# antonilo/unsupervised_detection

Measured on AMD Instinct MI355X. Metric: frame-pairs/sec per adversarial step, DAVIS 480p batch4, 1/2/4/8 GPU, higher is better.
Workload: dtype f32

## Files before the change

unsupervised_detection_amd/csrc/api_plan.hip:

```cpp
#include <stdlib.h>
#include <string.h>

#include "conv_host.h"
#include "elementwise.h"
#include "plan.h"

using namespace udet;

struct udet_plan {
  Plan* p;
};

extern "C" {

int udet_plan_create(const udet_config* c, udet_plan** out) {
  if (!c || !out) { set_error("plan_create: null argument"); return UDET_ERR_ARG; }
  Config k;
  k.batch = c->batch; k.in_h = c->in_h; k.in_w = c->in_w; k.img_h = c->img_h; k.img_w = c->img_w;
  k.flow_normalizer = c->flow_normalizer; k.cbn = c->cbn; k.epsilon = c->epsilon;
  k.lr = c->lr; k.beta1 = c->beta1; k.beta2 = c->beta2; k.adam_eps = c->adam_eps; k.clip = c->clip;
  k.noise_seed = c->noise_seed;
  k.conv_fp16 = c->conv_fp16 ? 1 : 0;
  Plan* P = plan_build(k);
  if (!P) return UDET_ERR_SHAPE;
// ... 53 lines not shown
}

int udet_pack_pwc(udet_plan* h, const float* w_pwc, void* ws, void* stream) {
  return plan_pack_pwc(h->p, w_pwc, (float*)ws, (hipStream_t)stream);
}
int udet_pack_trainable(udet_plan* h, const float* w_gen, const float* w_rec, void* ws, void* stream) {
  return plan_pack_trainable(h->p, w_gen, w_rec, (float*)ws, (hipStream_t)stream);
}
int udet_pwc_forward(udet_plan* h, const float* img1, const float* img2, void* ws, void* stream) {
  return plan_pwc_forward(h->p, img1, img2, (float*)ws, (hipStream_t)stream);
}
int udet_forward_from_flow(udet_plan* h, int ncalls, void* ws, void* stream) {
  UDET_TRY(plan_check_overflow(h->p, false));
  if (ncalls < 0 || ncalls > 3) { set_error("forward: ncalls must be 0..3"); return UDET_ERR_ARG; }
  return plan_forward(h->p, nullptr, nullptr, ncalls, (float*)ws, (hipStream_t)stream);
}
int udet_generator_forward(udet_plan* h, void* ws, void* stream) {
  UDET_TRY(plan_generator_forward(h->p, (float*)ws, (hipStream_t)stream));
  return plan_recover_forward(h->p, 0, (float*)ws, (hipStream_t)stream);
}
int udet_generator_layers(udet_plan* h, void* ws, void* stream) {
  h->p->ev_next = 0;
  UDET_TRY(plan_generator_layers(h->p, (float*)ws, (hipStream_t)stream));
  return plan_recover_forward(h->p, 0, (float*)ws, (hipStream_t)stream);
}
int udet_recover_forward(udet_plan* h, int n, void* ws, void* stream) {
  if (n < 1 || n > 3) { set_error("recover_forward: n must be 1..3 (multiples of the plan batch)"); return UDET_ERR_ARG; }
  return plan_recover_forward(h->p, n, (float*)ws, (hipStream_t)stream, true);
}
int udet_forward(udet_plan* h, const float* img1, const float* img2, int ncalls, void* ws, void* stream) {
  UDET_TRY(plan_check_overflow(h->p, false));
  if (ncalls < 0 || ncalls > 3) { set_error("forward: ncalls must be 0..3"); return UDET_ERR_ARG; }
  if (!img1 || !img2) { set_error("forward: null image pointer"); return UDET_ERR_ARG; }
  return plan_forward(h->p, img1, img2, ncalls, (float*)ws, (hipStream_t)stream);
}
int udet_prefetch_flow(udet_plan* h, const float* img1, const float* img2, void* ws, void* stream) {
  if (!img1 || !img2) { set_error("prefetch_flow: null image pointer"); return UDET_ERR_ARG; }
  return plan_prefetch(h->p, img1, img2, (float*)ws, (hipStream_t)stream);
}
int udet_prefetch_consume(udet_plan* h, void* ws, void* stream) {
  return plan_prefetch_consume(h->p, (float*)ws, (hipStream_t)stream);
}
int udet_forward_prefetched(udet_plan* h, int ncalls, void* ws, void* stream) {
  UDET_TRY(plan_check_overflow(h->p, false));
  if (ncalls < 0 || ncalls > 3) { set_error("forward: ncalls must be 0..3"); return UDET_ERR_ARG; }
  return plan_forward(h->p, nullptr, nullptr, ncalls, (float*)ws, (hipStream_t)stream, true);
}
int udet_backward(udet_plan* h, int which, const float* w_gen, const float* w_rec, float* g_gen, float* g_rec, void* ws,
                  void* stream) {
  UDET_TRY(plan_check_overflow(h->p, false));
  if (which < 1 || which > 3) { set_error("backward: which must be 1 (generator), 2 (recover) or 3 (both)"); return UDET_ERR_ARG; }
  return plan_backward(h->p, which, w_gen, w_rec, g_gen, g_rec, (float*)ws, (hipStream_t)stream);
}
int udet_apply(udet_plan* h, int net, float* w, float* g, float* m, float* v, void* ws, void* stream) {
  return plan_apply(h->p, net, w, g, m, v, (float*)ws, (hipStream_t)stream);
}
int udet_train_step(udet_plan* h, int which, const float* img1, const float* img2, float* w_gen, float* w_rec, float* g_gen,
                    float* g_rec, float* m_gen, float* v_gen, float* m_rec, float* v_rec, void* ws, void* stream) {
  UDET_TRY(udet_pack_trainable(h, w_gen, w_rec, ws, stream));
  UDET_TRY(udet_forward(h, img1, img2, 3, ws, stream));
  UDET_TRY(udet_backward(h, which, w_gen, w_rec, g_gen, g_rec, ws, stream));
  if (which & 1) UDET_TRY(udet_apply(h, NET_GEN, w_gen, g_gen, m_gen, v_gen, ws, stream));
  if (which & 2) UDET_TRY(udet_apply(h, NET_REC, w_rec, g_rec, m_rec, v_rec, ws, stream));
  return UDET_OK;
}

int udet_autotune(udet_plan* h, const float* w_gen, const float* w_rec, float* g_gen, float* g_rec, void* ws_, void* stream) {
  Plan* P = h->p;
  float* ws = (float*)ws_;
  hipStream_t s = (hipStream_t)stream;
  if (!P->pwc_packed) { set_error("autotune: pack the PWC-Net and trainable weights first"); return UDET_ERR_ARG; }
  const size_t lo = P->packed_floats, hi = P->small_off;
  UDET_TRY(launch_fill_uniform(ws + lo, (long)(hi - lo), 0x5eedull, -0.5f, 0.5f, s));
  const size_t img_floats = (size_t)P->cfg.batch * P->cfg.in_h * P->cfg.in_w * 3;
  if (P->wgrad_floats < 2 * img_floats) { set_error("autotune: workspace too small for the probe images"); return UDET_ERR_ARG; }
  const float* img1 = ws + P->wgrad_off[0];
  const float* img2 = img1 + img_floats;
  const bool was_concurrent = P->concurrent;
  P->concurrent = false;
  conv_set_tuning(1);
  wgrad_set_tuning(1);
  int rc = udet_forward(h, img1, img2, 3, ws_, stream);
  if (rc == UDET_OK) rc = udet_backward(h, 3, w_gen, w_rec, g_gen, g_rec, ws_, stream);
  conv_set_tuning(0);
  wgrad_set_tuning(0);
  P->concurrent = was_concurrent;
  UDET_HIP(hipMemsetAsync(ws + lo, 0, (hi - lo) * sizeof(float), s));
  UDET_HIP(hipStreamSynchronize(s));
  return rc;
}
int udet_tuned_shapes(void) { return tuned_shapes(); }
int udet_tune_save(const char* path) {
  FILE* f = path ? fopen(path, "w") : nullptr;
  if (!f) { set_error("tune_save: cannot open %s", path ? path : "(null)"); return UDET_ERR_ARG; }
  fprintf(f, "udet-tune 2 abi %d\n", UDET_TUNE_ABI);
  tune_dump(f);
  fclose(f);
  return UDET_OK;
}
int udet_tune_load(const char* path) {
  FILE* f = path ? fopen(path, "r") : nullptr;
  if (!f) { set_error("tune_load: cannot open %s", path ? path : "(null)"); return UDET_ERR_ARG; }
  char line[256];
  int n = 0, ver = 0, abi = -1;
  if (!fgets(line, sizeof(line), f) || sscanf(line, "udet-tune %d abi %d", &ver, &abi) != 2 || ver != 2 || abi != UDET_TUNE_ABI) {
    fclose(f);
    set_error("tune_load: %s is not a udet-tune 2 file of this build (abi %d)", path, UDET_TUNE_ABI);
    return UDET_ERR_ARG;
  }
  while (fgets(line, sizeof(line), f)) n += tune_put_line(line) ? 1 : 0;
  fclose(f);
  return n;
}

int udet_profile_begin(udet_plan* h) {
  for (auto* r : h->p->prof) delete r;
  h->p->prof.clear();
  h->p->profiling = true;
  return UDET_OK;
}
int udet_profile_end(udet_plan* h, double* out, int ncat, void* stream) {
  Plan* P = h->p;
  P->profiling = false;
  g_launch_sink = nullptr;
  UDET_HIP(hipStreamSynchronize((hipStream_t)stream));
  for (int i = 0; i < ncat * 5; ++i) out[i] = 0.0;
  FILE* dump = nullptr;
  if (const char* path = getenv("UDET_PROF_DUMP")) dump = fopen(path, "a");
  for (auto* r : P->prof) {
    float wall = 0.f;
    (void)hipEventElapsedTime(&wall, r->a, r->b);
    double kern = 0.0;
    std::string each;
    for (int k = 0; k < r->sink.n; ++k) {
      float ms = 0.f;
      if (hipEventElapsedTime(&ms, r->kev[2 * k], r->kev[2 * k + 1]) == hipSuccess) kern += ms;
      char buf[32];
      snprintf(buf, sizeof(buf), "%s%.1f", k ? "+" : "", ms * 1e3f);
      each += buf;
      (void)hipEventDestroy(r->kev[2 * k]);
      (void)hipEventDestroy(r->kev[2 * k + 1]);
    }
    if (r->sink.n == 0) kern = wall;
    if (dump)
      fprintf(dump, "%d,%s,%.4f,%.4f,%.4f,%.4f,%d,%s,%.4f\n", r->cat, r->name.c_str(), kern, r->flops * 1e-9, r->bytes * 1e-6, wall, r->sink.n,
              each.c_str(), r->flops * r->mfma_scale * 1e-9);
    if (r->cat < ncat) {
      out[r->cat * 5 + 0] += 1.0;
      out[r->cat * 5 + 1] += kern;
      out[r->cat * 5 + 2] += r->flops;
      out[r->cat * 5 + 3] += r->bytes;
      out[r->cat * 5 + 4] += wall;
    }
    (void)hipEventDestroy(r->a);
    (void)hipEventDestroy(r->b);
    delete r;
  }
  if (dump) fclose(dump);
  P->prof.clear();
  return UDET_OK;
}

int udet_generator_backward(udet_plan* h, const float* w_gen, float* g_gen, void* ws, void* stream) {
  if (!w_gen || !g_gen) { set_error("generator_backward: null argument"); return UDET_ERR_ARG; }
  return plan_backward(h->p, 1, w_gen, nullptr, g_gen, nullptr, (float*)ws, (hipStream_t)stream);
}
// ... 22 lines not shown
```

unsupervised_detection_amd/csrc/elementwise.h:

```cpp
#pragma once
#include "common.h"
namespace udet {
int launch_resize_bilinear_fwd(const float* x, int ldx, int x_coff, int N, int H, int W, float* y, int ldy, int y_coff,
                               int OH, int OW, int C, float mul, float div, hipStream_t s);
int launch_resize_bilinear_bwd(const float* dy, int ldy, int y_coff, int N, int OH, int OW, float* dx, int ldx, int x_coff,
                               int H, int W, int C, int accumulate, hipStream_t s);
int launch_upb_ring(const float* x, int ld, int N, int H, int W, float* xh, hipStream_t s);
int launch_upb_ring_fold(const float* dxh, int ld, int N, int H, int W, float* dx, hipStream_t s);
int launch_share_samples(float* buf, long P, int ld, int coff, int C, int copies, hipStream_t s);
int launch_fold_samples(float* buf, long P, int ld, int coff, int C, int copies, hipStream_t s);
int launch_emit_du(const float* d, const float* a, float* u, long P, int ld, int coff, int C, int act, float alpha, hipStream_t s);
int launch_pool2x2_sum(const float* du, float* dx, int N, int H, int W, int C, hipStream_t s);
int launch_pack_pwc_input(const float* i1, const float* i2, float* x8, long P, hipStream_t s);
int launch_gen_input(const float* img, const float* f, double* part, float* gin, int B, long HW, hipStream_t s);
size_t flow_stats_doubles(int B);
int launch_mask_rec_inputs(const float* logits, const float* f, float* mask, float* fin, long P, int ncalls, hipStream_t s);
int launch_pack_imgin(const float* img, float* imgin, long P, int ncalls, hipStream_t s);
int launch_losses(const float* f, const float* mask, const float* pred, long HW, int B, float cbn, float eps,
                  float num_pixels, float* part, float* losses, float* coef, float* sums, hipStream_t s);
size_t loss_part_floats(int B);
int launch_rec_loss_bwd(const float* f, const float* mask, const float* pred, float* dpred, long BHW, float cbn,
                        float inv_np, hipStream_t s);
int launch_gen_loss_bwd(const float* f, const float* mask, const float* pred, const float* coef, float* dpred,
                        float* dmask, long HW, int B, float cbn, hipStream_t s);
int launch_mask_bwd(const float* dmask, const float* dfin, const float* f, const float* mask, float* dlogits, long P,
                    hipStream_t s);
int launch_grad_absmean(const float* g, const long* seg_off, const long* seg_len, int nvars, float* vmean, float thresh,
                        float* out, hipStream_t s);
int launch_adam(float* w, float* g, float* m, float* v, long n, float lr_t, float b1, float b2, float eps, float clip,
                const float* flag, uint64_t seed, uint64_t step, hipStream_t s, int mode = 0, const int* skip = nullptr);
int launch_nonfinite_count(const float* g, long n, int* out, hipStream_t s);
int launch_flow_normalize(const float* f, double* part, float* out, int B, long HW, hipStream_t s);
int launch_charbonnier(const float* gt, const float* pred, const float* mask, int mc, int B, long HW, float cbn, float* part,
                       float* out, hipStream_t s);
int launch_crop_flip_resize(const void* src, int src_u8, int nearest, int N, int H, int W, int C, const int* prm, float* dst, int OH,
                            int OW, float div, float add, hipStream_t s);
int launch_crop_flip_resize_ragged(const void* src, int src_u8, int nearest, int N, int C, const long long* offsets, const int* hw,
                                   const int* prm, float* dst, int OH, int OW, float div, float add, hipStream_t s);
int launch_mask_stats(const float* pred, const float* gt, int N, int H, int W, float threshold, float gt_threshold, double* out,
                      hipStream_t s);
int launch_boundary_stats(const float* pred, const float* gt, const double* stats8, int N, int H, int W, float threshold,
                          float gt_threshold, int radius, unsigned long long* counts4, unsigned char* bmap_pred,
                          unsigned char* bmap_gt, hipStream_t s);
size_t restore_workspace_bytes(int n);
int launch_restore_masks_ragged(const float* masks, int n, int mh, int mw, const long long* offsets, const int* tab, const int* coef,
                                int max_h, int max_w, unsigned char* out, int* amax, unsigned char* binary, double threshold,
                                void* workspace, hipStream_t s);
size_t components_workspace_bytes(size_t total_pixels, int n);
int launch_select_components_ragged(const unsigned char* binary, const unsigned char* gt, int n, const long long* offsets, const int* hw,
                                    int max_h, int max_w, size_t total_pixels, int connectivity, int mode, int* labels,
                                    unsigned char* selected, long long* info, void* workspace, hipStream_t s);
size_t component_boxes_workspace_bytes(size_t total_pixels, int n);
int launch_component_boxes_ragged(const int* labels, const unsigned char* score, int n, const long long* offsets, const int* hw, int max_h,
                                  int max_w, size_t total_pixels, int min_area, int k, long long* dets, long long* counts, void* workspace,
                                  hipStream_t s);
int launch_draw_boxes_ragged(unsigned char* rgb, int n, const long long* offsets, const int* hw, const long long* dets,
                             const long long* counts, int k, int thickness, unsigned colour, hipStream_t s);
size_t link_detections_workspace_bytes(size_t total_pixels, int carry_h, int carry_w);
int launch_link_detections_ragged(const int* labels, int n, const long long* offsets, const int* hw, int max_h, int max_w,
                                  size_t total_pixels, const long long* dets, const long long* counts, int k, const int* link,
                                  const int* carry_labels, int carry_h, int carry_w, const long long* carry_dets,
                                  const long long* carry_counts, const int* carry_ids, const int* carry_next_id, int min_iou_permille,
                                  long long* inter, int* match, int* ids, int* linked, int* seq_tracks, int* next_id, void* workspace,
                                  hipStream_t s);
size_t link_detections_gap_workspace_bytes(size_t total_pixels, int m, int hist_h, int hist_w);
int launch_link_detections_gap_ragged(const int* labels, int n, const long long* offsets, const int* hw, int max_h, int max_w,
                                      size_t total_pixels, const long long* dets, const long long* counts, int k, const int* link,
                                      int max_gap, int m, const int* hist_labels, int hist_h, int hist_w, const long long* hist_dets,
                                      const long long* hist_counts, const int* hist_ids, int* hist_open, const int* hist_next_id,
                                      int min_iou_permille, long long* inter, int* match, int* ids, int* linked, int* seq_tracks,
                                      int* next_id, long long* gap_inter, int* back, int* prev, int* open, void* workspace,
                                      hipStream_t s);
int launch_draw_track_boxes_ragged(unsigned char* rgb, int n, const long long* offsets, const int* hw, const long long* dets,
                                   const long long* counts, int k, const int* ids, int thickness, const unsigned* palette,
                                   int palette_size, hipStream_t s);
int launch_fill_uniform(float* x, long n, uint64_t seed, float lo, float hi, hipStream_t s);
int launch_axpy(const float* x, float* y, long n, float a, int accumulate, hipStream_t s);
}
```

unsupervised_detection_amd/csrc/elementwise.hip:

```cpp
#include "common.h"
#include "elementwise.h"

namespace udet {

static inline int grid_for(long total, int cap = 4096) {
  long nb = (total + 255) / 256;
  if (nb > cap) nb = cap;
  if (nb < 1) nb = 1;
  return (int)nb;
}

template <typename T>
__device__ __forceinline__ T wave_sum(T v) {
#pragma unroll
  for (int o = 32; o > 0; o >>= 1) v += __shfl_down(v, o, 64);
  return v;
}
template <typename T>
__device__ __forceinline__ T block_sum(T v, T* sm ) {
  v = wave_sum(v);
  __syncthreads();
  if ((threadIdx.x & 63) == 0) sm[threadIdx.x >> 6] = v;
  __syncthreads();
  return sm[0] + sm[1] + sm[2] + sm[3];
// ... 521 lines not shown
  float red = 0.f, redc = 0.f, rs = 0.f;
  for (int b = 0; b < B; ++b) {
    float v[5] = {0, 0, 0, 0, 0};
    for (int k = 0; k < LS_BLOCKS; ++k)
      for (int j = 0; j < 5; ++j) v[j] += part[((long)b * LS_BLOCKS + k) * 5 + j];
    const float D = v[3] + eps, Dc = v[4] + eps;
    red += 1.f - v[0] / D;
    redc += 1.f - v[1] / Dc;
    rs += v[0] + v[1] + v[2];
    coef[b * 4 + 0] = -1.f / (B * D);
    coef[b * 4 + 1] = v[0] / (B * D * D);
    coef[b * 4 + 2] = -1.f / (B * Dc);
    coef[b * 4 + 3] = v[1] / (B * Dc * Dc);
    for (int j = 0; j < 5; ++j) sums[b * 5 + j] = v[j];
    if (b == 0) { losses[4] = v[0]; losses[5] = v[1]; losses[6] = D; losses[7] = Dc; }
  }
  red /= B; redc /= B;
  losses[0] = red + redc;
  losses[1] = rs / num_pixels;
  losses[2] = red;
  losses[3] = redc;
}
int launch_losses(const float* f, const float* mask, const float* pred, long HW, int B, float cbn, float eps,
                  float num_pixels, float* part, float* losses, float* coef, float* sums, hipStream_t s) {
  hipLaunchKernelGGL(loss_sums_kernel, dim3(LS_BLOCKS, B), dim3(256), 0, s, f, mask, pred, HW, B, cbn, part);
  hipLaunchKernelGGL(loss_finish_kernel, dim3(1), dim3(64), 0, s, part, B, eps, num_pixels, losses, coef, sums);
  UDET_HIP(hipGetLastError());
  return UDET_OK;
}
size_t loss_part_floats(int B) { return (size_t)B * LS_BLOCKS * 5; }

__global__ __launch_bounds__(256) void charbonnier_sum_kernel(const float* __restrict__ gt, const float* __restrict__ pred,
                                                              const float* __restrict__ mask, int mc, long HW, float cbn,
                                                              float* __restrict__ part ) {
  __shared__ float sm[4];
  const int n = blockIdx.y;
  float acc = 0.f;
  for (long p = (long)blockIdx.x * 256 + threadIdx.x; p < HW; p += (long)gridDim.x * 256) {
    const long q = (long)n * HW + p;
    const float2 a = *reinterpret_cast<const float2*>(gt + q * 2);
    const float2 b = *reinterpret_cast<const float2*>(pred + q * 2);
    const float m0 = mask ? mask[q * mc] : 1.f, m1 = mask ? mask[q * mc + (mc - 1)] : 1.f;
    acc += charb(a.x - b.x, cbn) * m0 + charb(a.y - b.y, cbn) * m1;
  }
  acc = block_sum(acc, sm);
  if (threadIdx.x == 0) part[(long)n * LS_BLOCKS + blockIdx.x] = acc;
}
__global__ void charbonnier_finish_kernel(const float* __restrict__ part, int B, float* __restrict__ out) {
  const int b = blockIdx.x * blockDim.x + threadIdx.x;
  if (b >= B) return;
  float v = 0.f;
  for (int k = 0; k < LS_BLOCKS; ++k) v += part[(long)b * LS_BLOCKS + k];
  out[b] = v;
}
int launch_charbonnier(const float* gt, const float* pred, const float* mask, int mc, int B, long HW, float cbn, float* part,
                       float* out, hipStream_t s) {
  hipLaunchKernelGGL(charbonnier_sum_kernel, dim3(LS_BLOCKS, B), dim3(256), 0, s, gt, pred, mask, mc, HW, cbn, part);
  hipLaunchKernelGGL(charbonnier_finish_kernel, dim3((B + 63) / 64), dim3(64), 0, s, part, B, out);
  UDET_HIP(hipGetLastError());
  return UDET_OK;
}

__global__ __launch_bounds__(256) void rec_loss_bwd_kernel(const float* __restrict__ f, const float* __restrict__ mask,
                                                           const float* __restrict__ pred, float* __restrict__ dpred,
                                                           long BHW, float cbn, float inv_np) {
  for (long q = (long)blockIdx.x * 256 + threadIdx.x; q < BHW; q += (long)gridDim.x * 256) {
    const float2 fl = *reinterpret_cast<const float2*>(f + q * 2);
    const float m = mask[q], cm = 1.f - m;
    const float2 a = *reinterpret_cast<const float2*>(pred + q * 2);
    const float2 b = *reinterpret_cast<const float2*>(pred + (BHW + q) * 2);
    const float2 c = *reinterpret_cast<const float2*>(pred + (2 * BHW + q) * 2);
    *reinterpret_cast<float2*>(dpred + q * 2) = make_float2(-charb_d(fl.x - a.x, cbn) * m * inv_np, -charb_d(fl.y - a.y, cbn) * m * inv_np);
    *reinterpret_cast<float2*>(dpred + (BHW + q) * 2) = make_float2(-charb_d(fl.x - b.x, cbn) * cm * inv_np, -charb_d(fl.y - b.y, cbn) * cm * inv_np);
    *reinterpret_cast<float2*>(dpred + (2 * BHW + q) * 2) = make_float2(-charb_d(fl.x - c.x, cbn) * inv_np, -charb_d(fl.y - c.y, cbn) * inv_np);
  }
}
int launch_rec_loss_bwd(const float* f, const float* mask, const float* pred, float* dpred, long BHW, float cbn,
                        float inv_np, hipStream_t s) {
  hipLaunchKernelGGL(rec_loss_bwd_kernel, dim3(grid_for(BHW)), dim3(256), 0, s, f, mask, pred, dpred, BHW, cbn, inv_np);
  UDET_HIP(hipGetLastError());
  return UDET_OK;
}

__global__ __launch_bounds__(256) void gen_loss_bwd_kernel(const float* __restrict__ f, const float* __restrict__ mask,
                                                           const float* __restrict__ pred, const float* __restrict__ coef,
                                                           float* __restrict__ dpred, float* __restrict__ dmask, long HW,
                                                           int B, float cbn) {
  const long BHW = (long)B * HW;
  for (long q = (long)blockIdx.x * 256 + threadIdx.x; q < BHW; q += (long)gridDim.x * 256) {
    const int n = (int)(q / HW);
    const float cR = coef[n * 4], cD = coef[n * 4 + 1], cRc = coef[n * 4 + 2], cDc = coef[n * 4 + 3];
    const float2 fl = *reinterpret_cast<const float2*>(f + q * 2);
    const float m = mask[q], cm = 1.f - m;
    const float2 a = *reinterpret_cast<const float2*>(pred + q * 2);
    const float2 b = *reinterpret_cast<const float2*>(pred + (BHW + q) * 2);
    const float2 c = *reinterpret_cast<const float2*>(pred + (2 * BHW + q) * 2);
    *reinterpret_cast<float2*>(dpred + q * 2) = make_float2(-cR * charb_d(fl.x - a.x, cbn) * m, -cR * charb_d(fl.y - a.y, cbn) * m);
    *reinterpret_cast<float2*>(dpred + (BHW + q) * 2) = make_float2(-cRc * charb_d(fl.x - b.x, cbn) * cm, -cRc * charb_d(fl.y - b.y, cbn) * cm);
    const float pa = charb(fl.x - a.x, cbn) + charb(fl.y - a.y, cbn);
    const float pb = charb(fl.x - b.x, cbn) + charb(fl.y - b.y, cbn);
    const float pc = charb(fl.x - c.x, cbn) + charb(fl.y - c.y, cbn);
    dmask[q] = cR * pa + cD * pc - cRc * pb - cDc * pc;
  }
}
int launch_gen_loss_bwd(const float* f, const float* mask, const float* pred, const float* coef, float* dpred,
                        float* dmask, long HW, int B, float cbn, hipStream_t s) {
  hipLaunchKernelGGL(gen_loss_bwd_kernel, dim3(grid_for((long)B * HW)), dim3(256), 0, s, f, mask, pred, coef, dpred, dmask,
                     HW, B, cbn);
  UDET_HIP(hipGetLastError());
  return UDET_OK;
}

__global__ __launch_bounds__(256) void mask_bwd_kernel(const float* __restrict__ dmask, const float* __restrict__ dfin,
                                                       const float* __restrict__ f, const float* __restrict__ mask,
                                                       float* __restrict__ dlogits , long P) {
  for (long q = (long)blockIdx.x * 256 + threadIdx.x; q < P; q += (long)gridDim.x * 256) {
    const float4 g0 = *reinterpret_cast<const float4*>(dfin + q * 4);
    const float4 g1 = *reinterpret_cast<const float4*>(dfin + (P + q) * 4);
    const float2 fl = *reinterpret_cast<const float2*>(f + q * 2);
    float dm = dmask[q];
    dm -= g0.x * fl.x + g0.y * fl.y + g0.w;
    dm += g1.x * fl.x + g1.y * fl.y + g1.w;
    const float m = mask[q];
    const float d0 = dm * m * (1.f - m) / 10.f;
    dlogits[q * 8] = d0;
    dlogits[q * 8 + 1] = -d0;
  }
}
int launch_mask_bwd(const float* dmask, const float* dfin, const float* f, const float* mask, float* dlogits, long P,
                    hipStream_t s) {
  hipLaunchKernelGGL(mask_bwd_kernel, dim3(grid_for(P)), dim3(256), 0, s, dmask, dfin, f, mask, dlogits, P);
  UDET_HIP(hipGetLastError());
  return UDET_OK;
}

#define GA_SPLIT 8
__global__ __launch_bounds__(256) void grad_absmean_kernel(const float* __restrict__ g, const long* __restrict__ seg_off,
                                                           const long* __restrict__ seg_len, float* __restrict__ vpart) {
  __shared__ float sm[4];
  const long off = seg_off[blockIdx.x], len = seg_len[blockIdx.x];
  const long b = len * blockIdx.y / GA_SPLIT, e = len * (blockIdx.y + 1) / GA_SPLIT;
  float s0 = 0.f, s1 = 0.f, s2 = 0.f, s3 = 0.f;
  long i = b + threadIdx.x;
  for (; i + 768 < e; i += 1024) {
    s0 += fabsf(g[off + i]);
    s1 += fabsf(g[off + i + 256]);
    s2 += fabsf(g[off + i + 512]);
    s3 += fabsf(g[off + i + 768]);
  }
  for (; i < e; i += 256) s0 += fabsf(g[off + i]);
  const float s = block_sum((s0 + s1) + (s2 + s3), sm);
  if (threadIdx.x == 0) vpart[blockIdx.x * GA_SPLIT + blockIdx.y] = s;
}
__global__ void grad_flag_kernel(const float* __restrict__ vpart, const long* __restrict__ seg_len, int nvars, float thresh,
                                 float* __restrict__ out ) {
  if (threadIdx.x == 0 && blockIdx.x == 0) {
    float s = 0.f;
    for (int i = 0; i < nvars; ++i) {
      float v = 0.f;
      for (int j = 0; j < GA_SPLIT; ++j) v += vpart[i * GA_SPLIT + j];
      s += v / (float)seg_len[i];
    }
    s /= (float)nvars;
    out[0] = s;
    out[1] = s < thresh ? 1.f : 0.f;
  }
}
int launch_grad_absmean(const float* g, const long* seg_off, const long* seg_len, int nvars, float* vmean, float thresh,
                        float* out, hipStream_t s) {
  hipLaunchKernelGGL(grad_absmean_kernel, dim3(nvars, GA_SPLIT), dim3(256), 0, s, g, seg_off, seg_len, vmean);
  hipLaunchKernelGGL(grad_flag_kernel, dim3(1), dim3(64), 0, s, vmean, seg_len, nvars, thresh, out);
  UDET_HIP(hipGetLastError());
  return UDET_OK;
}

__device__ __host__ __forceinline__ float udet_uniform01(uint64_t seed, uint64_t step, uint64_t idx) {
  uint64_t z = seed * 0x9E3779B97F4A7C15ull + step * 0xBF58476D1CE4E5B9ull + idx + 0x94D049BB133111EBull;
  z = (z ^ (z >> 30)) * 0xBF58476D1CE4E5B9ull;
  z = (z ^ (z >> 27)) * 0x94D049BB133111EBull;
  z = z ^ (z >> 31);
  return (float)(z >> 40) * (1.0f / 16777216.0f);
}

__global__ __launch_bounds__(256) void adam_kernel(float* __restrict__ w, float* __restrict__ g, float* __restrict__ m,
                                                   float* __restrict__ v, long n, float lr_t, float b1, float b2, float eps,
                                                   float clip, const float* __restrict__ flag, uint64_t seed,
                                                   uint64_t step, int mode, const int* __restrict__ skip) {
  if (skip && *skip != 0) return;
  const bool noise = flag && flag[1] != 0.f;
  for (long i = (long)blockIdx.x * 256 + threadIdx.x; i < n; i += (long)gridDim.x * 256) {
    float gi = g[i];
    if (mode != 2) {
      if (noise) gi = fabsf((udet_uniform01(seed, step, (uint64_t)i) * 2.f - 1.f) * clip);
      else gi = fminf(fmaxf(gi, -clip), clip);
      g[i] = gi;
      if (mode == 1) continue;
    }
    const float mi = m[i] + (gi - m[i]) * (1.f - b1);
    const float vi = v[i] + (gi * gi - v[i]) * (1.f - b2);
    m[i] = mi;
    v[i] = vi;
    w[i] = w[i] - lr_t * mi / (sqrtf(vi) + eps);
  }
}
__global__ __launch_bounds__(256) void fill_uniform_kernel(float* __restrict__ x, long n, uint64_t seed, float lo, float hi) {
  for (long i = (long)blockIdx.x * 256 + threadIdx.x; i < n; i += (long)gridDim.x * 256)
    x[i] = lo + (hi - lo) * udet_uniform01(seed, 0, (uint64_t)i);
}
int launch_fill_uniform(float* x, long n, uint64_t seed, float lo, float hi, hipStream_t s) {
  hipLaunchKernelGGL(fill_uniform_kernel, dim3(grid_for(n, 8192)), dim3(256), 0, s, x, n, seed, lo, hi);
  UDET_HIP(hipGetLastError());
  return UDET_OK;
}
__global__ __launch_bounds__(256) void mask_stats_kernel(const float* __restrict__ pred, const float* __restrict__ gt, int H, int W,
// ... 126 lines not shown
```

unsupervised_detection_amd/csrc/plan_step.hip:

```cpp
#include "conv_host.h"
#include "elementwise.h"
#include "plan_run.h"

namespace udet {

static const int PWC_CH[7] = {0, 16, 32, 64, 96, 128, 196};
static const char* const WARP_NAME[7] = {"", "", "warp_costvol2", "warp_costvol3", "warp_costvol4", "warp_costvol5", "warp_costvol6"};

static int pwc_forward_on(Plan* P, const float* img1, const float* img2, float* ws, const Lane& L0, const Lane& LH) {
  if (!P->pwc_packed) {
    set_error("pwc_forward: call udet_pack_pwc first");
    return UDET_ERR_ARG;
  }
  const Config& c = P->cfg;
  const Resolved& R = P->R;
  const int B = c.batch;
  hipStream_t s = L0.s;
  auto fwd = [&](int layer, int N, const Lane& ln) { return run_fwd(P, P->pwc[layer], N, ws, ln); };
  UDET_TRY(launch_pack_pwc_input(img1, img2, ws + P->buf(R.pwc_x8).off, (long)B * c.in_h * c.in_w, s));
  for (int l = 1; l <= 6; ++l)
    for (int j = 0; j < 3; ++j) UDET_TRY(fwd(R.pwc.pyr[l][j], 2 * B, L0));
  for (int l = 6; l >= 2; --l) {
    const int h = c.in_h >> l, w = c.in_w >> l, C = PWC_CH[l];
    const Buf& cb = P->buf(R.pwc_c[l]);
// ... 111 lines not shown
    for (int i = 0; i < 9; ++i) {
      const Layer& La = enc(0, i);
      UDET_TRY(run_fwd_pair(P, La, inputs_prepacked ? N : B, enc(1, i), N, ws, L0));
      if (!inputs_prepacked) UDET_TRY(share_enc_a_output(P, La, ncalls, ws, s));
    }
    P->enc_a_shared = !inputs_prepacked;
  } else {
    if (!skip_enc_a) {
      if (inputs_prepacked) {
        for (int i = 0; i < 9; ++i) UDET_TRY(run_fwd(P, enc(0, i), N, ws, L0));
        P->enc_a_shared = false;
      } else {
        UDET_TRY(plan_rec_image_branch(P, ncalls, ws, L0));
      }
    }
    for (int i = 0; i < 9; ++i) UDET_TRY(run_fwd(P, enc(1, i), N, ws, L0));
  }
  for (int k = 5; k >= 1; --k) {
    const Layer& dcl = P->rec[R.rec.deconv[k]];
    if (!dcl.upb) UDET_TRY(rec_resize(P, dec_src(R, k), R.rec_r[k + 1], N, ws, s));
    UDET_TRY(run_fwd(P, dcl, N, ws, L0));
    if (k < 5) {
      UDET_TRY(rec_resize(P, R.rec_flow[k + 1], R.rec_rf[k + 1], N, ws, s));
      UDET_TRY(run_fwd(P, P->rec[R.rec.upflow[k]], N, ws, L0));
    }
    UDET_TRY(run_fwd(P, P->rec[R.rec.flow[k]], N, ws, L0));
  }
  const Buf& f1 = P->buf(R.rec_flow[1]);
  return launch_resize_bilinear_fwd(ws + f1.off, f1.ld, 0, N, f1.h, f1.w, ws + P->buf(R.pred).off, 2, 0, c.img_h, c.img_w, 2, 1.f, 1.f, s);
}

int plan_losses(Plan* P, float* ws, hipStream_t s) {
  const Config& c = P->cfg;
  float* sm = ws + P->small_off;
  const long HW = (long)c.img_h * c.img_w;
  return launch_losses(ws + P->buf(P->R.flow).off, ws + P->buf(P->R.mask).off, ws + P->buf(P->R.pred).off, HW,
                       c.batch, c.cbn, c.epsilon, (float)(c.img_w * c.img_h * c.batch), sm + 8192, sm, sm + 16, sm + UDET_SMALL_SUMS, s);
}

int plan_prefetch_consume(Plan* P, float* ws, hipStream_t s) {
  if (!P->prefetch_pending) {
    set_error("forward_prefetched: no udet_prefetch_flow is pending");
    return UDET_ERR_ARG;
  }
  (void)hipStreamWaitEvent(s, P->prefetch_ev, 0);
  P->prefetch_pending = false;
  const Buf &fn = P->buf(P->R.flow_next), &in = P->buf(P->R.image_next);
  UDET_HIP(hipMemcpyAsync(ws + P->buf(P->R.flow).off, ws + fn.off, fn.floats() * sizeof(float), hipMemcpyDeviceToDevice, s));
  UDET_HIP(hipMemcpyAsync(ws + P->buf(P->R.image).off, ws + in.off, in.floats() * sizeof(float), hipMemcpyDeviceToDevice, s));
  return UDET_OK;
}

int plan_forward(Plan* P, const float* img1, const float* img2, int ncalls, float* ws, hipStream_t s, bool prefetched) {
  P->ev_next = 0;
  const Lane L0 = lane_of(P, s, 0), LI = lane_of(P, s, 1);
  if (prefetched) {
    UDET_TRY(plan_prefetch_consume(P, ws, s));
    img1 = img2 = nullptr;
  } else if (img1 && P->prefetch_pending) {
    (void)hipStreamWaitEvent(s, P->prefetch_ev, 0);
  }
  order_after(P, L0, LI);
  if (img1) UDET_TRY(plan_prepare_image(P, img1, P->R.image, ws, LI.s));
  hipEvent_t e_img = nullptr;
  if (LI.s != L0.s) {
    e_img = next_event(P);
    (void)hipEventRecord(e_img, LI.s);
  }
  const bool paired = pairs_on(P);
  UDET_TRY(plan_rec_image_branch(P, ncalls, ws, LI, !paired));
  if (img1) {
    UDET_TRY(pwc_forward_on(P, img1, img2, ws, L0, lane_of(P, s, 2)));
    UDET_TRY(plan_prepare_flow(P, P->R.flow, ws, s));
  }
  if (e_img) (void)hipStreamWaitEvent(s, e_img, 0);
  UDET_TRY(plan_generator_forward(P, ws, s));
  order_after(P, LI, L0);
  UDET_TRY(plan_recover_forward(P, ncalls, ws, s, false, !paired, paired));
  if (ncalls == 3) UDET_TRY(plan_losses(P, ws, s));
  return UDET_OK;
}

static int rec_backward(Plan* P, int N, const Resolved::Grad& G, bool with_wgrad, bool need_dfin, const float* w_rec, float* g_rec, float* ws,
                        const Lane& LD, const Lane& LW, const Lane* LAp = nullptr, const Lane* LWdecp = nullptr) {
  const Config& c = P->cfg;
  const Resolved& R = P->R;
  hipStream_t s = LD.s;
  const Lane LWdec = LWdecp ? *LWdecp : LW;
  auto wgrad_on = [&](const Lane& lw, const Layer& L, int dy, bool is_du, int n) -> int {
    order_after(P, LD, lw);
    return run_wgrad(P, L, n < 0 ? N : n, dy, is_du, w_rec, g_rec, ws, lw);
  };
  auto wgrad = [&](const Layer& L, int dy, bool is_du, int n = -1) -> int { return wgrad_on(LW, L, dy, is_du, n); };
  auto wgrad_dec = [&](const Layer& L, int dy, bool is_du) -> int { return wgrad_on(LWdec, L, dy, is_du, -1); };
  const Lane LA = LAp ? *LAp : LD;
  const bool a_own_lane = LA.s != LD.s;
  const int ncopies = N / c.batch;
  const bool a_shared = P->enc_a_shared && ncopies > 1;
  const Emit none;
  const float LEAK = 0.2f;
  {
    const Buf& df1 = P->buf(G.flow[1]);
    UDET_TRY(launch_resize_bilinear_bwd(ws + P->buf(G.pred).off, 2, 0, N, c.img_h, c.img_w, ws + df1.off, df1.ld, 0, df1.h, df1.w, 2, 0, s));
  }
  for (int k = 1; k <= 5; ++k) {
    const int dconcat = G.concat[k], uconcat = G.u_concat[k];
    const Layer* fl = &P->rec[R.rec.flow[k]];
    const Layer* dc = &P->rec[R.rec.deconv[k]];
    Emit em;
    em.ubuf = uconcat; em.abuf = fl->x; em.c0 = 0; em.c1 = dc->cout; em.act = ACT_LEAKY; em.alpha = LEAK;
    UDET_TRY(run_dgrad(P, *fl, N, G.flow[k], false, dconcat, 0, k == 1 ? 0 : 1, -1, em, ws, LD));
    if (with_wgrad) UDET_TRY(wgrad_dec(*fl, G.flow[k], false));
    if (k < 5) {
      const Layer* uf = &P->rec[R.rec.upflow[k]];
      if (with_wgrad) UDET_TRY(wgrad_dec(*uf, dconcat, false));
      UDET_TRY(run_dgrad(P, *uf, N, dconcat, false, G.rf[k + 1], 0, 0, -1, none, ws, LD));
      const Buf &drf = P->buf(G.rf[k + 1]), &dfn = P->buf(G.flow[k + 1]);
      UDET_TRY(launch_resize_bilinear_bwd(ws + drf.off, drf.ld, 0, N, drf.h, drf.w, ws + dfn.off, dfn.ld, 0, dfn.h, dfn.w, drf.ld, 0, s));
    }
    if (with_wgrad) {
      if (dc->upb) {
        order_after(P, LD, LWdec);
        UDET_TRY(rec_resize(P, dec_src(R, k), R.rec_r[k + 1], N, ws, LWdec.s));
      }
      UDET_TRY(wgrad_dec(*dc, uconcat, true));
    }
    if (dc->upb_bwd) {
      UDET_TRY(run_dgrad_upb(P, *dc, N, uconcat, G.p[k + 1], G.concat[k + 1], ws, LD));
      continue;
    }
    const int dr = G.r[k + 1];
    UDET_TRY(run_dgrad(P, *dc, N, uconcat, true, dr, 0, 0, -1, none, ws, LD));
    const Buf& bdr = P->buf(dr);
    const Buf& dsrc = P->buf(k == 5 ? G.conv6 : G.concat[k + 1]);
    UDET_TRY(launch_resize_bilinear_bwd(ws + bdr.off, bdr.ld, 0, N, bdr.h, bdr.w, ws + dsrc.off, dsrc.ld, 0, dsrc.h, dsrc.w,
                                        bdr.ld, 0, s));
  }
  {
    const Buf &d6 = P->buf(G.conv6), &a6 = P->buf(R.rec_conv6), &u6 = P->buf(G.u_conv6);
    UDET_TRY(launch_emit_du(ws + d6.off, ws + a6.off, ws + u6.off, (long)N * d6.h * d6.w, d6.ld, 0, d6.ld, ACT_LEAKY, LEAK, s));
  }
  if (a_own_lane) order_after(P, LD, LA);
  const bool pair_enc = pairs_on(P, 1) && with_wgrad && !a_own_lane;
  for (int i = 8; i >= 0; --i) {
    DgradJob job[2];
    int njob = 0;
    for (int e = 0; e < 2; ++e) {
      if (e == 0 && !with_wgrad) continue;
      const Layer* L = &P->rec[R.rec.enc[e][i]];
      const int du = G.enc_du[e][i];
      const bool shared = e == 0 && a_shared;
      const int Ne = shared ? c.batch : N;
      const bool own = e == 0 && a_own_lane;
      const Lane& LE = own ? LA : LD;
      hipStream_t se = LE.s;
      if (shared && i == 8) {
        const Buf& u = P->buf(du);
        UDET_TRY(launch_fold_samples(ws + u.off, (long)c.batch * u.h * u.w, u.ld, L->y_coff, L->cout, ncopies, se));
      }
      if (with_wgrad) {
        if (own) UDET_TRY(run_wgrad(P, *L, Ne, du, true, w_rec, g_rec, ws, LA));
        else UDET_TRY(wgrad(*L, du, true, Ne));
      }
      if (i == 0) {
        if (e == 1 && need_dfin) UDET_TRY(run_dgrad(P, *L, N, du, true, G.fin, 0, 0, -1, none, ws, LD));
        continue;
      }
      const int dx = G.enc_dx[e][i];
      const bool slab_in = L->x_in_slab;
      Emit em;
      em.ubuf = G.enc_ux[e][i]; em.abuf = L->x; em.c0 = 0; em.c1 = L->cin; em.act = ACT_LEAKY; em.alpha = LEAK;
      if (shared && slab_in) {
        const Buf& d = P->buf(dx);
        UDET_TRY(launch_fold_samples(ws + d.off, (long)c.batch * d.h * d.w, d.ld, L->x_coff, L->cin, ncopies, se));
      }
      if (pair_enc) {
        job[njob].L = L; job[njob].N = Ne; job[njob].dy = du; job[njob].dx = dx; job[njob].dx_coff = L->x_coff;
        job[njob].accumulate = slab_in ? 1 : 0; job[njob].em = em;
        ++njob;
        continue;
      }
      UDET_TRY(run_dgrad(P, *L, Ne, du, true, dx, L->x_coff, slab_in ? 1 : 0, -1, em, ws, LE));
    }
    if (njob == 2) UDET_TRY(run_dgrad_pair(P, job[0], job[1], ws, LD));
    else if (njob == 1) UDET_TRY(run_dgrad(P, *job[0].L, job[0].N, job[0].dy, true, job[0].dx, job[0].dx_coff, job[0].accumulate, -1, job[0].em, ws, LD));
  }
  if (a_own_lane) order_after(P, LA, LD);
  if (with_wgrad && LWdec.s != LW.s) order_after(P, LWdec, LD);
  return UDET_OK;
}

static int backward_recover(Plan* P, const float* w_rec, float* g_rec, float* ws, const Lane& LD, const Lane& LW, const Lane* LA = nullptr,
                            const Lane* LWdec = nullptr) {
  const Config& c = P->cfg;
  const Resolved& R = P->R;
  const long BHW = (long)c.batch * c.img_h * c.img_w;
  UDET_TRY(launch_rec_loss_bwd(ws + P->buf(R.flow).off, ws + P->buf(R.mask).off, ws + P->buf(R.pred).off, ws + P->buf(R.grad[0].pred).off, BHW,
                               c.cbn, 1.0f / (float)(c.img_w * c.img_h * c.batch), LD.s));
  return rec_backward(P, 3 * c.batch, R.grad[0], true, false, w_rec, g_rec, ws, LD, LW, LA, LWdec);
}

static int backward_generator(Plan* P, const float* w_gen, float* g_gen, float* ws, const Lane& LD, const Lane& LW, const Lane* LWlate = nullptr,
                              int nlate = 0) {
  const Config& c = P->cfg;
  const Resolved& R = P->R;
  const int B = c.batch;
  const long HW = (long)c.img_h * c.img_w;
  hipStream_t s = LD.s;
  float* sm = ws + P->small_off;
  UDET_TRY(launch_gen_loss_bwd(ws + P->buf(R.flow).off, ws + P->buf(R.mask).off, ws + P->buf(R.pred).off, sm + 16,
                               ws + P->buf(R.grad[1].pred).off, ws + P->buf(R.d_mask).off, HW, B, c.cbn, s));
  UDET_TRY(rec_backward(P, 2 * B, R.grad[1], false, true, nullptr, nullptr, ws, LD, LD));
  UDET_TRY(launch_mask_bwd(ws + P->buf(R.d_mask).off, ws + P->buf(R.grad[1].fin).off, ws + P->buf(R.flow).off, ws + P->buf(R.mask).off,
                           ws + P->buf(R.gen_d[17]).off, B * HW, s));
  for (int i = 16; i >= 0; --i) {
    const Layer& L = P->gen[i];
    const bool has_act = L.act != ACT_NONE;
    const int dy = has_act ? R.gen_u[i + 1] : R.gen_d[i + 1];
    const Lane& LWi = (LWlate && i < nlate) ? *LWlate : LW;
    order_after(P, LD, LWi);
    UDET_TRY(run_wgrad(P, L, B, dy, has_act, w_gen, g_gen, ws, LWi));
    if (i == 0) break;
    const int res = i == 6 ? R.gen_d[11] : (i == 3 ? R.gen_d[14] : (i == 1 ? R.gen_d[15] : -1));
    const int dx = R.gen_d[i];
    const Layer& Lp = P->gen[i - 1];
    const int ap = Lp.y2 >= 0 ? Lp.y2 : Lp.y;
    {
      Emit em;
      if (Lp.act != ACT_NONE) { em.ubuf = R.gen_u[i]; em.abuf = ap; em.c0 = 0; em.c1 = L.cin; em.act = Lp.act; em.alpha = Lp.alpha; }
      UDET_TRY(run_dgrad(P, L, B, dy, has_act, dx, 0, 0, res, em, ws, LD));
    }
  }
  return UDET_OK;
}

int plan_backward(Plan* P, int which, const float* w_gen, const float* w_rec, float* g_gen, float* g_rec, float* ws, hipStream_t s) {
  P->ev_next = 0;
  const Lane L0 = lane_of(P, s, 0), L1 = lane_of(P, s, 1), L2 = lane_of(P, s, 2), L3 = lane_of(P, s, 3);
  auto mark = [&](int net) {
    if (!P->grad_ev[net]) (void)hipEventCreateWithFlags(&P->grad_ev[net], hipEventDisableTiming);
    (void)hipEventRecord(P->grad_ev[net], s);
  };
  if (which == 3) {
    order_after(P, L0, L1);
    const int la = (int)plan_knob(UDET_KNOB_ENC_A_LANE);
    const Lane LA = lane_of(P, s, la > 0 && la < Plan::NLANE ? la : 0);
    const int lw = (int)plan_knob(UDET_KNOB_REC_DEC_WGRAD_LANE), le = (int)plan_knob(UDET_KNOB_REC_ENC_WGRAD_LANE);
    const Lane LWD = lane_of(P, s, lw > 0 && lw < Plan::NLANE ? lw : 3);
    const Lane LWE = lane_of(P, s, le > 0 && le < Plan::NLANE ? le : 2);
    UDET_TRY(backward_recover(P, w_rec, g_rec, ws, L0, LWE, la > 0 ? &LA : nullptr, &LWD));
    if (LWE.s != L2.s) order_after(P, LWE, L0);
    const long kl = plan_knob(UDET_KNOB_GEN_WGRAD_LATE);
    const int nlate = kl > 0 ? (int)kl : (kl < 0 ? 0 : 4);
    order_after(P, L2, L0);
    mark(NET_REC);
    UDET_TRY(backward_generator(P, w_gen, g_gen, ws, L1, L3, nlate > 0 ? &L2 : nullptr, nlate));
    order_after(P, L2, L0);
    order_after(P, L1, L0);
    order_after(P, L3, L0);
    mark(NET_GEN);
  } else if (which == 2) {
    UDET_TRY(backward_recover(P, w_rec, g_rec, ws, L0, L2, nullptr, &L3));
    order_after(P, L2, L0);
    mark(NET_REC);
  } else {
    UDET_TRY(backward_generator(P, w_gen, g_gen, ws, L0, L3));
    order_after(P, L3, L0);
    mark(NET_GEN);
  }
  return UDET_OK;
}

}
```

Baseline: 501.4.

## Reuse recover-net input gradient for generator backward instead of second rec backward pass

In the joint adversarial step (which==3), the recover network's backward pass now also computes the input-gradient dgrad for the first 2B samples and signals a lane. The generator backward then reuses that gradient, rescaled per sample by the loss coefficients, through a new mask_bwd_scaled kernel. This removes the separate full rec_backward pass over 2B samples and skips writing dpred in the generator loss kernel. It depends on the gradients being linearly related by the coef/inv_np scaling, and it adds cross-lane ordering. Autotune now also runs a generator-only backward so the shapes that path still uses get tuned.

```diff
diff --git a/unsupervised_detection_amd/csrc/api_plan.hip b/unsupervised_detection_amd/csrc/api_plan.hip
--- a/unsupervised_detection_amd/csrc/api_plan.hip
+++ b/unsupervised_detection_amd/csrc/api_plan.hip
@@ -159,6 +159,7 @@
   wgrad_set_tuning(1);
   int rc = udet_forward(h, img1, img2, 3, ws_, stream);
   if (rc == UDET_OK) rc = udet_backward(h, 3, w_gen, w_rec, g_gen, g_rec, ws_, stream);
+  if (rc == UDET_OK) rc = udet_backward(h, 1, w_gen, w_rec, g_gen, g_rec, ws_, stream);
   conv_set_tuning(0);
   wgrad_set_tuning(0);
   P->concurrent = was_concurrent;
diff --git a/unsupervised_detection_amd/csrc/elementwise.h b/unsupervised_detection_amd/csrc/elementwise.h
--- a/unsupervised_detection_amd/csrc/elementwise.h
+++ b/unsupervised_detection_amd/csrc/elementwise.h
@@ -25,6 +25,8 @@
                         float* dmask, long HW, int B, float cbn, hipStream_t s);
 int launch_mask_bwd(const float* dmask, const float* dfin, const float* f, const float* mask, float* dlogits, long P,
                     hipStream_t s);
+int launch_mask_bwd_scaled(const float* dmask, const float* dfin, const float* coef, float inv_np, const float* f, const float* mask,
+                           float* dlogits, long HW, int B, hipStream_t s);
 int launch_grad_absmean(const float* g, const long* seg_off, const long* seg_len, int nvars, float* vmean, float thresh,
                         float* out, hipStream_t s);
 int launch_adam(float* w, float* g, float* m, float* v, long n, float lr_t, float b1, float b2, float eps, float clip,
diff --git a/unsupervised_detection_amd/csrc/elementwise.hip b/unsupervised_detection_amd/csrc/elementwise.hip
--- a/unsupervised_detection_amd/csrc/elementwise.hip
+++ b/unsupervised_detection_amd/csrc/elementwise.hip
@@ -627,6 +627,7 @@
   return UDET_OK;
 }
 
+template <bool WITH_DPRED>
 __global__ __launch_bounds__(256) void gen_loss_bwd_kernel(const float* __restrict__ f, const float* __restrict__ mask,
                                                            const float* __restrict__ pred, const float* __restrict__ coef,
                                                            float* __restrict__ dpred, float* __restrict__ dmask, long HW,
@@ -640,8 +641,10 @@
     const float2 a = *reinterpret_cast<const float2*>(pred + q * 2);
     const float2 b = *reinterpret_cast<const float2*>(pred + (BHW + q) * 2);
     const float2 c = *reinterpret_cast<const float2*>(pred + (2 * BHW + q) * 2);
-    *reinterpret_cast<float2*>(dpred + q * 2) = make_float2(-cR * charb_d(fl.x - a.x, cbn) * m, -cR * charb_d(fl.y - a.y, cbn) * m);
-    *reinterpret_cast<float2*>(dpred + (BHW + q) * 2) = make_float2(-cRc * charb_d(fl.x - b.x, cbn) * cm, -cRc * charb_d(fl.y - b.y, cbn) * cm);
+    if (WITH_DPRED) {
+      *reinterpret_cast<float2*>(dpred + q * 2) = make_float2(-cR * charb_d(fl.x - a.x, cbn) * m, -cR * charb_d(fl.y - a.y, cbn) * m);
+      *reinterpret_cast<float2*>(dpred + (BHW + q) * 2) = make_float2(-cRc * charb_d(fl.x - b.x, cbn) * cm, -cRc * charb_d(fl.y - b.y, cbn) * cm);
+    }
     const float pa = charb(fl.x - a.x, cbn) + charb(fl.y - a.y, cbn);
     const float pb = charb(fl.x - b.x, cbn) + charb(fl.y - b.y, cbn);
     const float pc = charb(fl.x - c.x, cbn) + charb(fl.y - c.y, cbn);
@@ -650,8 +653,8 @@
 }
 int launch_gen_loss_bwd(const float* f, const float* mask, const float* pred, const float* coef, float* dpred,
                         float* dmask, long HW, int B, float cbn, hipStream_t s) {
-  hipLaunchKernelGGL(gen_loss_bwd_kernel, dim3(grid_for((long)B * HW)), dim3(256), 0, s, f, mask, pred, coef, dpred, dmask,
-                     HW, B, cbn);
+  if (dpred) hipLaunchKernelGGL(gen_loss_bwd_kernel<true>, dim3(grid_for((long)B * HW)), dim3(256), 0, s, f, mask, pred, coef, dpred, dmask, HW, B, cbn);
+  else hipLaunchKernelGGL(gen_loss_bwd_kernel<false>, dim3(grid_for((long)B * HW)), dim3(256), 0, s, f, mask, pred, coef, dpred, dmask, HW, B, cbn);
   UDET_HIP(hipGetLastError());
   return UDET_OK;
 }
@@ -675,6 +678,32 @@
 int launch_mask_bwd(const float* dmask, const float* dfin, const float* f, const float* mask, float* dlogits, long P,
                     hipStream_t s) {
   hipLaunchKernelGGL(mask_bwd_kernel, dim3(grid_for(P)), dim3(256), 0, s, dmask, dfin, f, mask, dlogits, P);
+  UDET_HIP(hipGetLastError());
+  return UDET_OK;
+}
+__global__ __launch_bounds__(256) void mask_bwd_scaled_kernel(const float* __restrict__ dmask, const float* __restrict__ dfin,
+                                                              const float* __restrict__ coef, float inv_np, const float* __restrict__ f,
+                                                              const float* __restrict__ mask, float* __restrict__ dlogits , long HW,
+                                                              int B) {
+  const long P = (long)B * HW;
+  for (long q = (long)blockIdx.x * 256 + threadIdx.x; q < P; q += (long)gridDim.x * 256) {
+    const int n = (int)(q / HW);
+    const float s0 = coef[n * 4] / inv_np, s1 = coef[n * 4 + 2] / inv_np;
+    const float4 g0 = *reinterpret_cast<const float4*>(dfin + q * 4);
+    const float4 g1 = *reinterpret_cast<const float4*>(dfin + (P + q) * 4);
+    const float2 fl = *reinterpret_cast<const float2*>(f + q * 2);
+    float dm = dmask[q];
+    dm -= s0 * (g0.x * fl.x + g0.y * fl.y + g0.w);
+    dm += s1 * (g1.x * fl.x + g1.y * fl.y + g1.w);
+    const float m = mask[q];
+    const float d0 = dm * m * (1.f - m) / 10.f;
+    dlogits[q * 8] = d0;
+    dlogits[q * 8 + 1] = -d0;
+  }
+}
+int launch_mask_bwd_scaled(const float* dmask, const float* dfin, const float* coef, float inv_np, const float* f, const float* mask,
+                           float* dlogits, long HW, int B, hipStream_t s) {
+  hipLaunchKernelGGL(mask_bwd_scaled_kernel, dim3(grid_for((long)B * HW)), dim3(256), 0, s, dmask, dfin, coef, inv_np, f, mask, dlogits, HW, B);
   UDET_HIP(hipGetLastError());
   return UDET_OK;
 }
diff --git a/unsupervised_detection_amd/csrc/plan_step.hip b/unsupervised_detection_amd/csrc/plan_step.hip
--- a/unsupervised_detection_amd/csrc/plan_step.hip
+++ b/unsupervised_detection_amd/csrc/plan_step.hip
@@ -217,7 +217,8 @@
 }
 
 static int rec_backward(Plan* P, int N, const Resolved::Grad& G, bool with_wgrad, bool need_dfin, const float* w_rec, float* g_rec, float* ws,
-                        const Lane& LD, const Lane& LW, const Lane* LAp = nullptr, const Lane* LWdecp = nullptr) {
+                        const Lane& LD, const Lane& LW, const Lane* LAp = nullptr, const Lane* LWdecp = nullptr, int Nfin = -1,
+                        const Lane* Lfin = nullptr) {
   const Config& c = P->cfg;
   const Resolved& R = P->R;
   hipStream_t s = LD.s;
@@ -298,7 +299,10 @@
         else UDET_TRY(wgrad(*L, du, true, Ne));
       }
       if (i == 0) {
-        if (e == 1 && need_dfin) UDET_TRY(run_dgrad(P, *L, N, du, true, G.fin, 0, 0, -1, none, ws, LD));
+        if (e == 1 && need_dfin) {
+          UDET_TRY(run_dgrad(P, *L, Nfin < 0 ? N : Nfin, du, true, G.fin, 0, 0, -1, none, ws, LD));
+          if (Lfin) order_after(P, LD, *Lfin);
+        }
         continue;
       }
       const int dx = G.enc_dx[e][i];
@@ -325,18 +329,19 @@
   return UDET_OK;
 }
 
+static float rec_loss_inv_np(const Config& c) { return 1.0f / (float)(c.img_w * c.img_h * c.batch); }
 static int backward_recover(Plan* P, const float* w_rec, float* g_rec, float* ws, const Lane& LD, const Lane& LW, const Lane* LA = nullptr,
-                            const Lane* LWdec = nullptr) {
+                            const Lane* LWdec = nullptr, const Lane* Lfin = nullptr) {
   const Config& c = P->cfg;
   const Resolved& R = P->R;
   const long BHW = (long)c.batch * c.img_h * c.img_w;
   UDET_TRY(launch_rec_loss_bwd(ws + P->buf(R.flow).off, ws + P->buf(R.mask).off, ws + P->buf(R.pred).off, ws + P->buf(R.grad[0].pred).off, BHW,
-                               c.cbn, 1.0f / (float)(c.img_w * c.img_h * c.batch), LD.s));
-  return rec_backward(P, 3 * c.batch, R.grad[0], true, false, w_rec, g_rec, ws, LD, LW, LA, LWdec);
+                               c.cbn, rec_loss_inv_np(c), LD.s));
+  return rec_backward(P, 3 * c.batch, R.grad[0], true, Lfin != nullptr, w_rec, g_rec, ws, LD, LW, LA, LWdec, 2 * c.batch, Lfin);
 }
 
 static int backward_generator(Plan* P, const float* w_gen, float* g_gen, float* ws, const Lane& LD, const Lane& LW, const Lane* LWlate = nullptr,
-                              int nlate = 0) {
+                              int nlate = 0, bool fin_from_rec = false) {
   const Config& c = P->cfg;
   const Resolved& R = P->R;
   const int B = c.batch;
@@ -344,10 +349,15 @@
   hipStream_t s = LD.s;
   float* sm = ws + P->small_off;
   UDET_TRY(launch_gen_loss_bwd(ws + P->buf(R.flow).off, ws + P->buf(R.mask).off, ws + P->buf(R.pred).off, sm + 16,
-                               ws + P->buf(R.grad[1].pred).off, ws + P->buf(R.d_mask).off, HW, B, c.cbn, s));
-  UDET_TRY(rec_backward(P, 2 * B, R.grad[1], false, true, nullptr, nullptr, ws, LD, LD));
-  UDET_TRY(launch_mask_bwd(ws + P->buf(R.d_mask).off, ws + P->buf(R.grad[1].fin).off, ws + P->buf(R.flow).off, ws + P->buf(R.mask).off,
-                           ws + P->buf(R.gen_d[17]).off, B * HW, s));
+                               fin_from_rec ? nullptr : ws + P->buf(R.grad[1].pred).off, ws + P->buf(R.d_mask).off, HW, B, c.cbn, s));
+  if (fin_from_rec) {
+    UDET_TRY(launch_mask_bwd_scaled(ws + P->buf(R.d_mask).off, ws + P->buf(R.grad[0].fin).off, sm + 16, rec_loss_inv_np(c), ws + P->buf(R.flow).off,
+                                    ws + P->buf(R.mask).off, ws + P->buf(R.gen_d[17]).off, HW, B, s));
+  } else {
+    UDET_TRY(rec_backward(P, 2 * B, R.grad[1], false, true, nullptr, nullptr, ws, LD, LD));
+    UDET_TRY(launch_mask_bwd(ws + P->buf(R.d_mask).off, ws + P->buf(R.grad[1].fin).off, ws + P->buf(R.flow).off, ws + P->buf(R.mask).off,
+                             ws + P->buf(R.gen_d[17]).off, B * HW, s));
+  }
   for (int i = 16; i >= 0; --i) {
     const Layer& L = P->gen[i];
     const bool has_act = L.act != ACT_NONE;
@@ -383,13 +393,13 @@
     const int lw = (int)plan_knob(UDET_KNOB_REC_DEC_WGRAD_LANE), le = (int)plan_knob(UDET_KNOB_REC_ENC_WGRAD_LANE);
     const Lane LWD = lane_of(P, s, lw > 0 && lw < Plan::NLANE ? lw : 3);
     const Lane LWE = lane_of(P, s, le > 0 && le < Plan::NLANE ? le : 2);
-    UDET_TRY(backward_recover(P, w_rec, g_rec, ws, L0, LWE, la > 0 ? &LA : nullptr, &LWD));
+    UDET_TRY(backward_recover(P, w_rec, g_rec, ws, L0, LWE, la > 0 ? &LA : nullptr, &LWD, &L1));
     if (LWE.s != L2.s) order_after(P, LWE, L0);
     const long kl = plan_knob(UDET_KNOB_GEN_WGRAD_LATE);
     const int nlate = kl > 0 ? (int)kl : (kl < 0 ? 0 : 4);
     order_after(P, L2, L0);
     mark(NET_REC);
-    UDET_TRY(backward_generator(P, w_gen, g_gen, ws, L1, L3, nlate > 0 ? &L2 : nullptr, nlate));
+    UDET_TRY(backward_generator(P, w_gen, g_gen, ws, L1, L3, nlate > 0 ? &L2 : nullptr, nlate, true));
     order_after(P, L2, L0);
     order_after(P, L1, L0);
     order_after(P, L3, L0);
```

Result: no change. 501.8 (median of 6 runs) (+0.1%).
